# c976237222/HunyuanVideo_efficiency

Hardware: AMD Instinct MI355X
Metric: denoise-steps/sec (720x1280x129f, HunyuanVideo DiT 20+40 blocks, bf16) (higher is better)
Workload: dtype bf16

## Files before the change

hunyuanvideo_efficiency_amd/_lib.py:

```python
from __future__ import annotations

import ctypes as C
import os
import re

_HERE = os.path.dirname(os.path.abspath(__file__))
LIB_PATH = os.path.join(_HERE, "lib", "libhv_kernels.so")
TORCH_OPS_PATH = os.path.join(_HERE, "lib", "libhv_torch_ops.so")
ABI_VERSION = 5

_p, _i, _l, _f = C.c_void_p, C.c_int, C.c_int64, C.c_float

SIGNATURES = {
    "hv_abi_version": [],
    "hv_ln_modulate_bf16": [_p, _p, _p, _p, _l, _i, _l, _l, _f, _i, _p],
    "hv_qknorm_rope_bf16": [_p, _p, _p, _p, _p, _l, _l, _i, _i, _l, _l, _f, _p],
    "hv_qknorm_rope_scatter_bf16": [_p, _p, _p, _p, _p, _l, _l, _i, _i, _l, _l, _f, _p, _l, _i, _l, _p],
    "hv_gemm_bf16": [_p, _l, _p, _l, _p, _i, _i, _i, _p, _l, _i, _i, _p, _l, _i, _p, _p, _l, _p],
    "hv_linear_smallm_bf16": [_p, _p, _p, _p, _p, _i, _i, _i, _l, _l, _i, _p],
    "hv_timestep_embedding_bf16": [_p, _p, _i, _i, _f, _p],
    "hv_attn_fwd_bf16": [_p, _p, _p, _p, _l, _l, _l, _l, _i, _i, _i, _i, _f, _p, _l, _p],
    "hv_attn_workspace_bytes": [_i, _i, _i],
    "hv_attn_w4_loop_signature": [],
    "hv_attn_partial_bf16": [_p, _p, _p, _l, _l, _l, _i, _i, _i, _i, _f, _p, _p, _i, _i, _i, _p],
    "hv_attn_merge_bf16": [_p, _p, _p, _l, _i, _i, _i, _p],
    "hv_attn_suggest_splits": [_i, _i, _i],
    "hv_patchify_f32_bf16": [_p, _p, _i, _i, _i, _i, _p],
    "hv_unpatchify_bf16": [_p, _p, _i, _i, _i, _i, _l, _p],
    "hv_euler_step_f32": [_p, _p, _f, _l, _p],
    "hv_euler_step_f32_f32": [_p, _p, _f, _l, _p],
    "hv_masked_mean_bf16": [_p, _p, _p, _i, _i, _p],
    "hv_broadcast_row_bf16": [_p, _p, _l, _i, _l, _p],
    "hv_copy3d_bf16": [_p, _p, _i, _l, _i, _l, _l, _l, _l, _p],
    "hv_fp8_dequant_bf16": [_p, _p, _p, _l, _p],
    "hv_ln_modulate_fp8": [_p, _p, _p, _p, _p, _l, _i, _l, _l, _f, _p],
    "hv_quant_rows_fp8": [_p, _l, _p, _l, _p, _l, _i, _p],
    "hv_gemm_fp8": [_p, _l, _p, _p, _l, _p, _p, _i, _i, _i, _p, _l, _i, _i, _p, _l, _i, _p, _p, _l, _p],
    "hv_gemm_f16": [_p, _l, _p, _l, _p, _i, _i, _i, _p, _l, _i, _p, _l, _p],
    "hv_conv3d_causal_f16": [_p, _l, _p, _p, _p, _l, _i, _i, _i, _i, _i, _i, _i, _p, _l, _p, _l, _p],
    "hv_gn_partial_rows": [_l],
    "hv_subpixel_gn_partial_rows": [_i, _i, _i, _i],
    "hv_groupnorm_finalize_f16": [_p, _l, _l, _l, _i, _i, _f, _p, _p, _p, _p],
    "hv_groupnorm_affine_f16": [_p, _l, _l, _i, _i, _f, _p, _p, _p, _l, _p, _p],
    "hv_groupnorm_apply_f16": [_p, _l, _p, _l, _l, _i, _p, _i, _p],
    "hv_softmax_rows_f32_f16": [_p, _l, _p, _l, _i, _i, _i, _f, _i, _p],
# ... 91 lines not shown
```

hunyuanvideo_efficiency_amd/csrc/hv_attention.hip:

```cpp
#include "hv_attention.hpp"

using namespace hv_attn;

namespace {

constexpr int QTILE = 256;

__global__ __launch_bounds__(256) void attn_combine_kernel(const float* __restrict__ part_o, const float* __restrict__ part_ml,
                                                            bf16_t* __restrict__ o, int64_t so, int n_q, int n_heads, int n_splits) {
    const int64_t idx = (int64_t)blockIdx.x * blockDim.x + threadIdx.x;
    const int64_t total = (int64_t)n_q * n_heads * 32;
    if (idx >= total) return;
    const int d4 = (int)(idx & 31);
    const int64_t rh = idx >> 5;
    const int head = (int)(rh % n_heads);
    const int64_t row = rh / n_heads;
    float m = -INFINITY;
    for (int s = 0; s < n_splits; ++s) m = fmaxf(m, part_ml[(((int64_t)s * n_q + row) * n_heads + head) * 2]);
    float4 acc = make_float4(0.f, 0.f, 0.f, 0.f);
    float l = 0.f;
    for (int s = 0; s < n_splits; ++s) {
        const int64_t ri = ((int64_t)s * n_q + row) * n_heads + head;
        const float w = __builtin_amdgcn_exp2f(part_ml[ri * 2] - m);
        const float4 v = *reinterpret_cast<const float4*>(part_o + ri * D + d4 * 4);
        acc.x += v.x * w; acc.y += v.y * w; acc.z += v.z * w; acc.w += v.w * w;
        l += part_ml[ri * 2 + 1] * w;
    }
    const float inv = 1.0f / l;
    u32x2 w2;
    w2[0] = pack_bf2(acc.x * inv, acc.y * inv);
    w2[1] = pack_bf2(acc.z * inv, acc.w * inv);
    *reinterpret_cast<u32x2*>(o + row * so + head * D + d4 * 4) = w2;
}

int attn_launch(const AttnArgs& a, dim3 grid, hipStream_t stream) { return launch_w4(a, grid, stream); }

constexpr int KMAX_ROWS = 2048;
__global__ __launch_bounds__(256) void attn_kmax_kernel(const bf16_t* __restrict__ k, int64_t sk, int n_kv, unsigned* __restrict__ out) {
    __shared__ float wmax[4];
    const int head = blockIdx.y, t = threadIdx.x, ch = t & 15;
    const int r0 = blockIdx.x * KMAX_ROWS, r1 = min(r0 + KMAX_ROWS, n_kv);
    float best = 0.f;
    for (int row = r0 + (t >> 4); row < r1; row += 16) {
        const u32x4 w = *reinterpret_cast<const u32x4*>(k + (int64_t)row * sk + head * D + ch * 8);
        float s = 0.f;
#pragma unroll
        for (int j = 0; j < 4; ++j) {
            const float lo = bf2f_lo(w[j]), hi = bf2f_hi(w[j]);
            s += lo * lo + hi * hi;
        }
#pragma unroll
        for (int o = 8; o > 0; o >>= 1) s += __shfl_xor(s, o, 64);
        best = fmaxf(best, s);
    }
    best = fmaxf(best, __shfl_xor(best, 16, 64));
    best = fmaxf(best, __shfl_xor(best, 32, 64));
    if ((t & 63) == 0) wmax[t >> 6] = best;
    __syncthreads();
    if (t == 0) atomicMax(out + head, __float_as_uint(fmaxf(fmaxf(wmax[0], wmax[1]), fmaxf(wmax[2], wmax[3]))));
}

int attn_prepare_kmax(AttnArgs& a, void* workspace, int64_t workspace_bytes, hipStream_t stream) {
    a.kmax2 = nullptr;
    if (!workspace || workspace_bytes < KMAX_BYTES || a.n_heads > KMAX_HEADS || a.n_kv < 64 * KVT) return HV_OK;
    if (hipMemsetAsync(workspace, 0, KMAX_BYTES, stream) != hipSuccess) return HV_ERR_LAUNCH;
    attn_kmax_kernel<<<dim3((unsigned)((a.n_kv + KMAX_ROWS - 1) / KMAX_ROWS), (unsigned)a.n_heads), dim3(256), 0, stream>>>(a.k, a.sk, a.n_kv, (unsigned*)workspace);
    a.kmax2 = (const unsigned*)workspace;
    return HV_OK;
}

}

extern "C" int64_t hv_attn_workspace_bytes(int n_q, int n_kv, int n_heads) {
    (void)n_kv;
    return (int64_t)KMAX_BYTES + (int64_t)2 * n_q * n_heads * (128 + 2) * (int64_t)sizeof(float);
}

extern "C" int hv_attn_fwd_bf16(const void* q, const void* k, const void* v, void* o, int64_t stride_q, int64_t stride_k,
                                int64_t stride_v, int64_t stride_o, int n_q, int n_kv, int n_heads, int head_dim,
                                float scale, void* workspace, int64_t workspace_bytes, hipStream_t stream) {
    if (!q || !k || !v || !o || head_dim != D || n_heads <= 0 || n_q < 0 || n_kv < 0 || (stride_q & 7) || (stride_k & 7) ||
        (stride_v & 7) || (stride_o & 3))
        return HV_ERR_ARG;
    if (n_q == 0) return HV_OK;
    if (n_kv == 0) return HV_ERR_ARG;
    AttnArgs a;
    a.q = (const bf16_t*)q; a.k = (const bf16_t*)k; a.v = (const bf16_t*)v; a.o = (bf16_t*)o;
    a.sq = stride_q; a.sk = stride_k; a.sv = stride_v; a.so = stride_o;
    a.n_q = n_q; a.n_kv = n_kv; a.n_heads = n_heads;
    a.n_qtiles = (n_q + QTILE - 1) / QTILE;
    a.scale_log2e = scale * 1.4426950408889634f;
    a.n_splits = 1; a.split_keys = n_kv; a.part_o = nullptr; a.part_ml = nullptr; a.partial = 0;
    if (attn_prepare_kmax(a, workspace, workspace_bytes, stream) != HV_OK) return HV_ERR_LAUNCH;
    {
        const int64_t nwg = (int64_t)a.n_qtiles * n_heads;
        const int ntile = (n_kv + KVT - 1) / KVT;
        const double r1 = (double)((nwg + 255) / 256), r2 = 0.5 * (double)((2 * nwg + 255) / 256);
        if (workspace && ntile >= 64 && r2 < 0.97 * r1 && workspace_bytes >= hv_attn_workspace_bytes(n_q, n_kv, n_heads)) {
            a.n_splits = 2;
            a.split_keys = ((ntile + 1) / 2) * KVT;
            a.part_o = (float*)((char*)workspace + KMAX_BYTES);
            a.part_ml = a.part_o + (int64_t)2 * n_q * n_heads * D;
        }
    }
    if (attn_launch(a, dim3((unsigned)(a.n_qtiles * n_heads), (unsigned)a.n_splits), stream) != HV_OK) return HV_ERR_LAUNCH;
    if (a.n_splits > 1) {
        const int64_t total = (int64_t)n_q * n_heads * 32;
        attn_combine_kernel<<<dim3((unsigned)((total + 255) / 256)), dim3(256), 0, stream>>>(a.part_o, a.part_ml, a.o, a.so, n_q, n_heads,
                                                                                           a.n_splits);
    }
    return hv_check_launch();
}

extern "C" int hv_attn_partial_bf16(const void* q, const void* k, const void* v, int64_t stride_q, int64_t stride_k, int64_t stride_v,
                                    int n_q, int n_kv, int n_heads, int head_dim, float scale, void* part_o, void* part_ml,
                                    int n_slots, int slot, int splits, hipStream_t stream) {
    if (!q || !k || !v || !part_o || !part_ml || head_dim != D || n_heads <= 0 || n_q < 0 || n_kv <= 0 || (stride_q & 7) ||
        (stride_k & 7) || (stride_v & 7) || (splits != 1 && splits != 2) || slot < 0 || slot + splits > n_slots)
        return HV_ERR_ARG;
    if (n_q == 0) return HV_OK;
    const int ntile = (n_kv + KVT - 1) / KVT;
    if (splits == 2 && ntile < 2) return HV_ERR_ARG;
    AttnArgs a;
    a.q = (const bf16_t*)q; a.k = (const bf16_t*)k; a.v = (const bf16_t*)v; a.o = nullptr;
    a.sq = stride_q; a.sk = stride_k; a.sv = stride_v; a.so = 0;
    a.n_q = n_q; a.n_kv = n_kv; a.n_heads = n_heads;
    a.n_qtiles = (n_q + QTILE - 1) / QTILE;
    a.scale_log2e = scale * 1.4426950408889634f;
    a.n_splits = splits;
    a.split_keys = splits == 2 ? ((ntile + 1) / 2) * KVT : n_kv;
    a.part_o = (float*)part_o + (int64_t)slot * n_q * n_heads * D;
    a.part_ml = (float*)part_ml + (int64_t)slot * n_q * n_heads * 2;
    a.partial = 1;
    a.kmax2 = nullptr;
    if (attn_launch(a, dim3((unsigned)(a.n_qtiles * n_heads), (unsigned)splits), stream) != HV_OK) return HV_ERR_LAUNCH;
    return hv_check_launch();
}

extern "C" int hv_attn_merge_bf16(const void* part_o, const void* part_ml, void* o, int64_t stride_o, int n_q, int n_heads, int n_slots,
                                  hipStream_t stream) {
    if (!part_o || !part_ml || !o || n_heads <= 0 || n_q < 0 || n_slots <= 0 || (stride_o & 3)) return HV_ERR_ARG;
    if (n_q == 0) return HV_OK;
    const int64_t total = (int64_t)n_q * n_heads * 32;
    attn_combine_kernel<<<dim3((unsigned)((total + 255) / 256)), dim3(256), 0, stream>>>((const float*)part_o, (const float*)part_ml,
                                                                                       (bf16_t*)o, stride_o, n_q, n_heads, n_slots);
    return hv_check_launch();
}

extern "C" int hv_attn_suggest_splits(int n_q, int n_kv, int n_heads) {
    const int64_t nwg = (int64_t)((n_q + QTILE - 1) / QTILE) * n_heads;
    const int ntile = (n_kv + KVT - 1) / KVT;
    const double r1 = (double)((nwg + 255) / 256), r2 = 0.5 * (double)((2 * nwg + 255) / 256);
    return (ntile >= 64 && r2 < 0.97 * r1) ? 2 : 1;
}
```

hunyuanvideo_efficiency_amd/csrc/hv_attention.hpp:

```cpp
#pragma once
#include "hv_common.hpp"
#include "../../include/hv_kernels.h"
#include <type_traits>

namespace hv_attn {

constexpr int D = 128;
constexpr int KVT = 64;
constexpr int KV_TILE_BYTES = KVT * D * 2;

struct AttnArgs {
    const bf16_t* q; const bf16_t* k; const bf16_t* v; bf16_t* o;
    int64_t sq, sk, sv, so;
    int n_q, n_kv, n_heads, n_qtiles;
    float scale_log2e;
    int n_splits, split_keys;
    float* part_o;
    float* part_ml;
    int partial;
    const unsigned* kmax2;
};
constexpr int KMAX_BYTES = 256;
constexpr int KMAX_HEADS = 62;

typedef __attribute__((ext_vector_type(4))) short s16x4;
typedef __attribute__((address_space(3))) s16x4* lds_s16x4_ptr;
typedef __attribute__((address_space(3))) void* lds_void_ptr;

__device__ __forceinline__ float half_swap_max(float v) {
    auto r = __builtin_amdgcn_permlane32_swap(__float_as_uint(v), __float_as_uint(v), false, false);
    return fmaxf(__uint_as_float(r[0]), __uint_as_float(r[1]));
}
__device__ __forceinline__ float half_swap_sum(float v) {
    auto r = __builtin_amdgcn_permlane32_swap(__float_as_uint(v), __float_as_uint(v), false, false);
    return __uint_as_float(r[0]) + __uint_as_float(r[1]);
}

template <int I, int N, typename F>
__device__ __forceinline__ void static_for(F&& f) {
    if constexpr (I < N) {
        f(std::integral_constant<int, I>{});
        static_for<I + 1, N>(f);
    }
}

int launch_w4(const AttnArgs& a, dim3 grid, hipStream_t stream);

}
```

hunyuanvideo_efficiency_amd/csrc/hv_attention_w4.hip:

```cpp
#include "hv_attention.hpp"
#include "hv_agpr_clobbers.inc"

using namespace hv_attn;

namespace {

constexpr int W4_WAVES = 4, W4_QTILE = 256, W4_NBUF = 4;
constexpr int W4_KOFF = 0, W4_VOFF = W4_NBUF * KV_TILE_BYTES;
constexpr int W4_LDS = 2 * W4_NBUF * KV_TILE_BYTES;
constexpr int A_O = 0, A_Q = 128, A_KF = 192, A_VF = 224;
constexpr int RING = 8;
constexpr int PF = 4;
constexpr int WGRP = 2;
__host__ __device__ constexpr int frag_insts(int f) { return (f >= 16 && f < 32) ? 2 : 1; }
__host__ __device__ constexpr int wait_for(int f) { int n = 0; for (int i = WGRP; i < PF; ++i) n += frag_insts(f + i); return n; }

template <int KF, int QF, int WAIT>
__device__ __forceinline__ void mfma_s_first(f32x16& s, const f32x16& c) {
    if constexpr (WAIT >= 0)
        asm volatile("s_waitcnt lgkmcnt(%c6)\n\tv_mfma_f32_32x32x16_bf16 %0, a[%c2:%c3], a[%c4:%c5], %1"
                     : "=&v"(s) : "v"(c), "i"(KF), "i"(KF + 3), "i"(QF), "i"(QF + 3), "i"(WAIT) : HV_CLOBBER_ALL_AGPRS);
    else
        asm volatile("v_mfma_f32_32x32x16_bf16 %0, a[%c2:%c3], a[%c4:%c5], %1"
                     : "=&v"(s) : "v"(c), "i"(KF), "i"(KF + 3), "i"(QF), "i"(QF + 3) : HV_CLOBBER_ALL_AGPRS);
// ... 34 lines not shown
__device__ __forceinline__ void add_pinned(float& acc, float p) { asm volatile("v_add_f32 %0, %0, %1" : "+v"(acc) : "v"(p)); }
__device__ __forceinline__ void exp2_pinned(float& d, float x) { asm volatile("v_exp_f32 %0, %1" : "=v"(d) : "v"(x)); }
__device__ __forceinline__ void pack_pinned(uint32_t& w, float lo, float hi) { asm volatile("v_cvt_pk_bf16_f32 %0, %1, %2" : "=v"(w) : "v"(lo), "v"(hi)); }
__device__ __forceinline__ void max3_pinned(float& acc, float x, float y) { asm volatile("v_max3_f32 %0, %0, %1, %2" : "+v"(acc) : "v"(x), "v"(y)); }
template <int N>
__device__ __forceinline__ void acc_write(uint32_t v) { asm volatile("v_accvgpr_write_b32 a%c1, %0" : : "v"(v), "i"(N)); }
template <int N>
__device__ __forceinline__ float acc_read() {
    float v;
    asm volatile("v_accvgpr_read_b32 %0, a%c1" : "=v"(v) : "i"(N));
    return v;
}

#include "hv_attention_w4_loop.inc"

__host__ __device__ constexpr int exps_before(int g) { return g <= 32 ? g + (g + 3) / 4 : (g <= 56 ? 40 + (g - 32) : 64); }
__host__ __device__ constexpr int exps_in(int g) { return exps_before(g + 1) - exps_before(g); }

__global__ __launch_bounds__(256, 1) void attn_fwd_kernel_w4(AttnArgs a) {
#if defined(__HIP_DEVICE_COMPILE__)
    extern __shared__ __attribute__((aligned(16))) char smem[];
    const int tid = threadIdx.x, lane = tid & 63, wave = tid >> 6;
    const int lr = lane & 31, lh = lane >> 5;
    const int head = blockIdx.x / a.n_qtiles;
    const int qt = blockIdx.x % a.n_qtiles;
    if (a.n_splits > 1) {
        const int kv0 = blockIdx.y * a.split_keys;
        a.k += (int64_t)kv0 * a.sk;
        a.v += (int64_t)kv0 * a.sv;
        a.n_kv = min(a.n_kv - kv0, a.split_keys);
    }
    const int q0 = qt * W4_QTILE + wave * 64;
    const uint32_t lds0 = (uint32_t)(uintptr_t)smem;

    asm volatile("; hv_attention_w4: a[0:255] owned by inline asm" : : : HV_CLOBBER_ALL_AGPRS);
    static_for<0, 128>([&](auto I) { asm volatile("v_accvgpr_write_b32 a%c0, 0" : : "i"(A_O + decltype(I)::value)); });
    float qn2[2] = {0.f, 0.f};
#pragma unroll
    for (int qb = 0; qb < 2; ++qb) {
        const int qrow = min(q0 + qb * 32 + lr, a.n_q - 1);
        const bf16_t* qp = a.q + (int64_t)qrow * a.sq + head * D + lh * 8;
        u32x4 raw[8];
#pragma unroll
        for (int ks = 0; ks < 8; ++ks) raw[ks] = *reinterpret_cast<const u32x4*>(qp + ks * 16);
        static_for<0, 32>([&](auto I) {
            constexpr int i = decltype(I)::value;
            const uint32_t w = raw[i >> 2][i & 3];
            const uint32_t sc = pack_bf2(bf2f_lo(w) * a.scale_log2e, bf2f_hi(w) * a.scale_log2e);
            qn2[qb] += bf2f_lo(sc) * bf2f_lo(sc) + bf2f_hi(sc) * bf2f_hi(sc);
            if (qb == 0) acc_write<A_Q + i>(sc);
            else acc_write<A_Q + 32 + i>(sc);
        });
    }

// ... 340 lines not shown
                }
        asm volatile("s_nop 1" : "+v"(pw[0][0]), "+v"(pw[0][1]), "+v"(pw[0][2]), "+v"(pw[0][3]), "+v"(pw[1][0]), "+v"(pw[1][1]), "+v"(pw[1][2]),
                     "+v"(pw[1][3]));
        static_for<0, 16>([&](auto F) {
            constexpr int f = decltype(F)::value, kk = f >> 2, db = f & 3, VF = A_VF + 4 * (f % RING);
            lds_v<VF, kk * 16 * 256>(vv[db]);
            static_for<0, 2>([&](auto QB) {
                constexpr int qb = decltype(QB)::value;
                mfma_pv<A_O + 16 * (qb * 4 + db), VF, (qb == 0 ? 0 : -1)>(pw[qb][kk]);
            });
        });
        l_run[0] += ls[0];
        l_run[1] += ls[1];
    }
    asm volatile("s_nop 7\n\ts_nop 7\n\ts_nop 7" ::: "memory");

#pragma unroll
    for (int qb = 0; qb < 2; ++qb) {
        float o[64];
        if (qb == 0) static_for<0, 64>([&](auto I) { o[decltype(I)::value] = acc_read<A_O + decltype(I)::value>(); });
        else static_for<0, 64>([&](auto I) { o[decltype(I)::value] = acc_read<A_O + 64 + decltype(I)::value>(); });
        const float l_tot = half_swap_sum(l_run[qb]);
        const int qrow = q0 + qb * 32 + lr;
        if (a.n_splits > 1 || a.partial) {
            if (qrow < a.n_q) {
                const int64_t rowi = ((int64_t)blockIdx.y * a.n_q + qrow) * a.n_heads + head;
                float* po = a.part_o + rowi * D + 4 * lh;
#pragma unroll
                for (int db = 0; db < 4; ++db)
#pragma unroll
                    for (int g = 0; g < 4; ++g)
                        *reinterpret_cast<float4*>(po + db * 32 + g * 8) =
                            make_float4(o[db * 16 + 4 * g], o[db * 16 + 4 * g + 1], o[db * 16 + 4 * g + 2], o[db * 16 + 4 * g + 3]);
                if (lh == 0) {
                    a.part_ml[rowi * 2] = m_run[qb];
                    a.part_ml[rowi * 2 + 1] = l_tot;
                }
            }
        } else if (qrow < a.n_q) {
            const float inv = 1.0f / l_tot;
            bf16_t* op = a.o + (int64_t)qrow * a.so + head * D + 4 * lh;
#pragma unroll
            for (int db = 0; db < 4; ++db)
#pragma unroll
                for (int g = 0; g < 4; ++g) {
                    u32x2 w;
                    w[0] = pack_bf2(o[db * 16 + 4 * g] * inv, o[db * 16 + 4 * g + 1] * inv);
                    w[1] = pack_bf2(o[db * 16 + 4 * g + 2] * inv, o[db * 16 + 4 * g + 3] * inv);
                    *reinterpret_cast<u32x2*>(op + db * 32 + g * 8) = w;
                }
        }
    }
#endif
}

HvPerDeviceOnce g_w4_lds_once;

}

extern "C" int hv_attn_w4_loop_signature(void) { return (int)HV_W4_LOOP_SIGNATURE; }

int hv_attn::launch_w4(const AttnArgs& a, dim3 grid, hipStream_t stream) {
    if (hv_set_max_lds(g_w4_lds_once, (const void*)attn_fwd_kernel_w4, W4_LDS) != HV_OK) return HV_ERR_LAUNCH;
    attn_fwd_kernel_w4<<<grid, dim3(256), W4_LDS, stream>>>(a);
    return HV_OK;
}
```

hunyuanvideo_efficiency_amd/csrc/hv_torch_ops.cpp:

```cpp
#include <torch/library.h>
#include <ATen/core/Tensor.h>
#include <c10/hip/HIPStream.h>
#include <c10/hip/HIPGuard.h>
#include <optional>
#include <vector>
#include "../../include/hv_kernels.h"

namespace {
using OptT = std::optional<at::Tensor>;

struct Dev {
    c10::DeviceIndex idx = -1;
    const char* op;
    explicit Dev(const char* o) : op(o) {}
    void* p(const OptT& t, const char* name) {
        if (!t.has_value() || !t->defined()) return nullptr;
        TORCH_CHECK(t->is_cuda(), "hv::", op, ": ", name, " must be a GPU tensor (this library has no CPU path), got ", t->device());
        if (idx < 0) idx = t->device().index();
        TORCH_CHECK(t->device().index() == idx, "hv::", op, ": ", name, " is on a different GPU than the other tensors");
        return t->data_ptr();
    }
};

inline void check_rc(int rc, const char* op) {
// ... 78 lines not shown
    TORCH_CHECK(dev.idx >= 0, "hv::timestep_embedding_bf16: needs at least one GPU tensor");
    c10::hip::HIPGuard guard(dev.idx);
    hipStream_t stream = c10::hip::getCurrentHIPStream(dev.idx).stream();
    check_rc(hv_timestep_embedding_bf16(a0, a1, (int)n_t, (int)dim, (float)max_period, stream), "timestep_embedding_bf16");
}

void op_attn_fwd_bf16(const OptT& q, const OptT& k, const OptT& v, const OptT& o, int64_t stride_q, int64_t stride_k, int64_t stride_v, int64_t stride_o, int64_t n_q, int64_t n_kv, int64_t n_heads, int64_t head_dim, double scale, const OptT& workspace, int64_t workspace_bytes) {
    Dev dev("attn_fwd_bf16");
    auto a0 = (const void*)dev.p(q, "q");
    auto a1 = (const void*)dev.p(k, "k");
    auto a2 = (const void*)dev.p(v, "v");
    auto a3 = (void*)dev.p(o, "o");
    auto a13 = (void*)dev.p(workspace, "workspace");
    TORCH_CHECK(dev.idx >= 0, "hv::attn_fwd_bf16: needs at least one GPU tensor");
    c10::hip::HIPGuard guard(dev.idx);
    hipStream_t stream = c10::hip::getCurrentHIPStream(dev.idx).stream();
    check_rc(hv_attn_fwd_bf16(a0, a1, a2, a3, (int64_t)stride_q, (int64_t)stride_k, (int64_t)stride_v, (int64_t)stride_o, (int)n_q, (int)n_kv, (int)n_heads, (int)head_dim, (float)scale, a13, (int64_t)workspace_bytes, stream), "attn_fwd_bf16");
}

int64_t op_attn_workspace_bytes(int64_t n_q, int64_t n_kv, int64_t n_heads) {
    return (int64_t)hv_attn_workspace_bytes((int)n_q, (int)n_kv, (int)n_heads);
}

int64_t op_attn_w4_loop_signature() {
    return (int64_t)hv_attn_w4_loop_signature();
}

void op_attn_partial_bf16(const OptT& q, const OptT& k, const OptT& v, int64_t stride_q, int64_t stride_k, int64_t stride_v, int64_t n_q, int64_t n_kv, int64_t n_heads, int64_t head_dim, double scale, const OptT& part_o, const OptT& part_ml, int64_t n_slots, int64_t slot, int64_t splits) {
    Dev dev("attn_partial_bf16");
    auto a0 = (const void*)dev.p(q, "q");
    auto a1 = (const void*)dev.p(k, "k");
    auto a2 = (const void*)dev.p(v, "v");
    auto a11 = (void*)dev.p(part_o, "part_o");
    auto a12 = (void*)dev.p(part_ml, "part_ml");
    TORCH_CHECK(dev.idx >= 0, "hv::attn_partial_bf16: needs at least one GPU tensor");
    c10::hip::HIPGuard guard(dev.idx);
    hipStream_t stream = c10::hip::getCurrentHIPStream(dev.idx).stream();
    check_rc(hv_attn_partial_bf16(a0, a1, a2, (int64_t)stride_q, (int64_t)stride_k, (int64_t)stride_v, (int)n_q, (int)n_kv, (int)n_heads, (int)head_dim, (float)scale, a11, a12, (int)n_slots, (int)slot, (int)splits, stream), "attn_partial_bf16");
}

void op_attn_merge_bf16(const OptT& part_o, const OptT& part_ml, const OptT& o, int64_t stride_o, int64_t n_q, int64_t n_heads, int64_t n_slots) {
    Dev dev("attn_merge_bf16");
    auto a0 = (const void*)dev.p(part_o, "part_o");
    auto a1 = (const void*)dev.p(part_ml, "part_ml");
    auto a2 = (void*)dev.p(o, "o");
    TORCH_CHECK(dev.idx >= 0, "hv::attn_merge_bf16: needs at least one GPU tensor");
// ... 314 lines not shown

void op_vae_postprocess_f16_f32(const OptT& x, const OptT& out, int64_t n) {
    Dev dev("vae_postprocess_f16_f32");
    auto a0 = (const void*)dev.p(x, "x");
    auto a1 = (float*)dev.p(out, "out");
    TORCH_CHECK(dev.idx >= 0, "hv::vae_postprocess_f16_f32: needs at least one GPU tensor");
    c10::hip::HIPGuard guard(dev.idx);
    hipStream_t stream = c10::hip::getCurrentHIPStream(dev.idx).stream();
    check_rc(hv_vae_postprocess_f16_f32(a0, a1, (int64_t)n, stream), "vae_postprocess_f16_f32");
}

}

TORCH_LIBRARY(hv, m) {
    m.def("abi_version() -> int");
    m.def("ln_modulate_bf16(Tensor? x, Tensor? shift_or_bias, Tensor? scale_or_weight, Tensor(a!)? out, int M, int D, int ldx, int ldo, float eps, int mode) -> ()");
    m.def("qknorm_rope_bf16(Tensor(a!)? qkv, Tensor? q_weight, Tensor? k_weight, Tensor? cos_tab, Tensor? sin_tab, int n_rows, int n_rope, int n_heads, int head_dim, int ld, int k_offset, float eps) -> ()");
    m.def("qknorm_rope_scatter_bf16(Tensor? qkv, Tensor? q_weight, Tensor? k_weight, Tensor? cos_tab, Tensor? sin_tab, int n_rows, int n_rope, int n_heads, int head_dim, int ld, int k_offset, float eps, Tensor(a!)? dst, int dst_ld, int heads_per_block, int dst_block_stride) -> ()");
    m.def("gemm_bf16(Tensor? A, int lda, Tensor? W, int ldw, Tensor? bias, int M, int N, int K, Tensor(a!)? out0, int ld0, int act0, int n_split, Tensor(b!)? out1, int ld1, int act1, Tensor? gate, Tensor? res, int ld_res) -> ()");
    m.def("linear_smallm_bf16(Tensor? x, Tensor? W, Tensor? bias, Tensor? addend, Tensor(a!)? out, int M, int N, int K, int ldx, int ldo, int act) -> ()");
    m.def("timestep_embedding_bf16(Tensor? t, Tensor(a!)? out, int n_t, int dim, float max_period) -> ()");
    m.def("attn_fwd_bf16(Tensor? q, Tensor? k, Tensor? v, Tensor(a!)? o, int stride_q, int stride_k, int stride_v, int stride_o, int n_q, int n_kv, int n_heads, int head_dim, float scale, Tensor(b!)? workspace, int workspace_bytes) -> ()");
    m.def("attn_workspace_bytes(int n_q, int n_kv, int n_heads) -> int");
    m.def("attn_w4_loop_signature() -> int");
    m.def("attn_partial_bf16(Tensor? q, Tensor? k, Tensor? v, int stride_q, int stride_k, int stride_v, int n_q, int n_kv, int n_heads, int head_dim, float scale, Tensor(a!)? part_o, Tensor(b!)? part_ml, int n_slots, int slot, int splits) -> ()");
    m.def("attn_merge_bf16(Tensor? part_o, Tensor? part_ml, Tensor(a!)? o, int stride_o, int n_q, int n_heads, int n_slots) -> ()");
    m.def("attn_suggest_splits(int n_q, int n_kv, int n_heads) -> int");
    m.def("patchify_f32_bf16(Tensor? x, Tensor(a!)? A, int C, int T, int H, int W) -> ()");
    m.def("unpatchify_bf16(Tensor? y, Tensor(a!)? out, int C, int T, int H, int W, int ldy) -> ()");
    m.def("euler_step_f32(Tensor(a!)? sample, Tensor? model_out_bf16, float dt, int n) -> ()");
    m.def("euler_step_f32_f32(Tensor(a!)? sample, Tensor? model_out_f32, float dt, int n) -> ()");
    m.def("masked_mean_bf16(Tensor? x, Tensor? mask, Tensor(a!)? out, int L, int D) -> ()");
    m.def("broadcast_row_bf16(Tensor? src, Tensor(a!)? dst, int n_rows, int D, int ld) -> ()");
    m.def("copy3d_bf16(Tensor? src, Tensor(a!)? dst, int n_batch, int rows, int cols, int src_batch_stride, int src_ld, int dst_batch_stride, int dst_ld) -> ()");
    m.def("fp8_dequant_bf16(Tensor? w_e4m3fn, Tensor? scale_bf16, Tensor(a!)? out_bf16, int n) -> ()");
    m.def("ln_modulate_fp8(Tensor? x, Tensor? shift, Tensor? scale, Tensor(a!)? out_q, Tensor(b!)? out_row_scale, int M, int D, int ldx, int ldq, float eps) -> ()");
    m.def("quant_rows_fp8(Tensor? x, int ldx, Tensor(a!)? out_q, int ldq, Tensor(b!)? out_row_scale, int M, int K) -> ()");
    m.def("gemm_fp8(Tensor? A_q, int lda, Tensor? a_row_scale, Tensor? W_q, int ldw, Tensor? w_scale_bf16, Tensor? bias, int M, int N, int K, Tensor(a!)? out0, int ld0, int act0, int n_split, Tensor(b!)? out1, int ld1, int act1, Tensor? gate, Tensor? res, int ld_res) -> ()");
    m.def("gemm_f16(Tensor? A, int lda, Tensor? W, int ldw, Tensor? bias, int M, int N, int K, Tensor(a!)? out, int ldo, int out_is_f32, Tensor? res, int ld_res) -> ()");
    m.def("conv3d_causal_f16(Tensor? x, int ldx, Tensor? w_taps, Tensor? bias, Tensor(a!)? out, int ldo, int T, int H, int W, int Cin, int Cout, int up_t, int up_hw, Tensor? res, int ld_res, Tensor(b!)? gn_partial, int gn_partial_floats) -> ()");
    m.def("gn_partial_rows(int M) -> int");
    m.def("subpixel_gn_partial_rows(int sT, int sH, int sW, int up_t) -> int");
    m.def("conv3d_upsampled_subpixel_f16(Tensor? x, int ldx, Tensor? w_sub, Tensor? tap_table, int ntap, Tensor? bias, Tensor(a!)? out, int ldo, int sT, int sH, int sW, int Cin, int Cout, int up_t, Tensor(b!)? gn_partial, int gn_partial_floats) -> ()");
    m.def("conv3d_cout4_f16(Tensor? x, int ldx, Tensor? affine, int silu, Tensor? w_frag, Tensor? bias, Tensor(a!)? out, int ldo, int T, int H, int W, int Cin, int Cout, Tensor(b!)? planes, int planes_floats) -> ()");
    m.def("conv3d_cout4_planes_floats(int M) -> int");
    m.def("conv3d_causal_strided_f16(Tensor? x, int ldx, Tensor? w_taps, Tensor? bias, Tensor(a!)? out, int ldo, int sT, int sH, int sW, int Cin, int Cout, int stride_t, int stride_h, int stride_w) -> ()");
// ... 30 lines not shown
    m.impl("ln_modulate_fp8", &op_ln_modulate_fp8);
    m.impl("quant_rows_fp8", &op_quant_rows_fp8);
    m.impl("gemm_fp8", &op_gemm_fp8);
    m.impl("gemm_f16", &op_gemm_f16);
    m.impl("conv3d_causal_f16", &op_conv3d_causal_f16);
    m.impl("conv3d_upsampled_subpixel_f16", &op_conv3d_upsampled_subpixel_f16);
    m.impl("conv3d_cout4_f16", &op_conv3d_cout4_f16);
    m.impl("conv3d_causal_strided_f16", &op_conv3d_causal_strided_f16);
    m.impl("temporal_resample_f16", &op_temporal_resample_f16);
    m.impl("groupnorm_affine_f16", &op_groupnorm_affine_f16);
    m.impl("groupnorm_finalize_f16", &op_groupnorm_finalize_f16);
    m.impl("groupnorm_apply_f16", &op_groupnorm_apply_f16);
    m.impl("softmax_rows_f32_f16", &op_softmax_rows_f32_f16);
    m.impl("transpose_16b", &op_transpose_16b);
    m.impl("vae_latent_tile_f16", &op_vae_latent_tile_f16);
    m.impl("vae_blend_f16", &op_vae_blend_f16);
    m.impl("copy4d_16b", &op_copy4d_16b);
    m.impl("vae_postprocess_f16_f32", &op_vae_postprocess_f16_f32);
}

TORCH_LIBRARY_IMPL(hv, CompositeExplicitAutograd, m) {
    m.impl("abi_version", &op_abi_version);
    m.impl("attn_workspace_bytes", &op_attn_workspace_bytes);
    m.impl("attn_w4_loop_signature", &op_attn_w4_loop_signature);
    m.impl("attn_suggest_splits", &op_attn_suggest_splits);
    m.impl("gn_partial_rows", &op_gn_partial_rows);
    m.impl("subpixel_gn_partial_rows", &op_subpixel_gn_partial_rows);
    m.impl("conv3d_cout4_planes_floats", &op_conv3d_cout4_planes_floats);
}
```

hunyuanvideo_efficiency_amd/ops.py:

```python
from __future__ import annotations

from typing import Optional

import torch

from . import _lib

BF16 = torch.bfloat16
ACT_NONE, ACT_GELU_TANH, ACT_SILU = 0, 1, 2
PROFILE_ATTN = None


def _chk(t: torch.Tensor, dtype, name: str, last_contig: bool = True):
    if not t.is_cuda:
        raise _lib.HVKernelError(f"{name}: expected a GPU tensor (this package has no CPU path), got {t.device}")
    if t.dtype != dtype:
        raise TypeError(f"{name}: expected {dtype}, got {t.dtype}")
    if last_contig and t.dim() > 0 and t.stride(-1) != 1:
        raise ValueError(f"{name}: innermost dimension must be contiguous")


def _rows(t: torch.Tensor, name: str):
    if t.dim() == 1:
        return 1, t.shape[0], t.shape[0]
# ... 82 lines not shown
    assert k == kw and ldw == k and m <= 4
    if out is None:
        out = torch.empty(*x.shape[:-1], n, dtype=BF16, device=x.device)
    _, _, ldo = _rows(out, "out")
    if bias is not None:
        _chk(bias, BF16, "bias")
    if addend is not None:
        _chk(addend, BF16, "addend")
        assert addend.shape == out.shape and addend.stride() == out.stride()
    _lib.call("linear_smallm_bf16", x, w, bias, addend, out, m, n, k, ldx, ldo,
                                                 (1 if silu_in else 0) | (2 if silu_out else 0))
    return out


_attn_ws = {}


ATTN_MIN_WORKSPACE = 256


def _attn_workspace(n_q, n_kv, n_heads, device):
    if n_kv < 64 * 64:
        return None
    n_wg = ((n_q + 255) // 256) * n_heads
    need = ATTN_MIN_WORKSPACE if n_wg >= 16 * 256 else int(_lib.host("attn_workspace_bytes", n_q, n_kv, n_heads))
    key = str(device)
    ws = _attn_ws.get(key)
    if ws is None or ws.numel() < need:
        ws = torch.empty(need, dtype=torch.uint8, device=device)
        _attn_ws[key] = ws
    return ws


def attn_fwd(q, k, v, out, n_heads: int, scale: Optional[float] = None, kv_split_workspace: bool = True):
    for t, nm in ((q, "q"), (k, "k"), (v, "v"), (out, "out")):
        _chk(t, BF16, nm)
        assert t.dim() == 2
    n_q, n_kv = q.shape[0], k.shape[0]
    assert v.shape[0] == n_kv and out.shape[0] == n_q
    if scale is None:
        scale = 128 ** -0.5
    prof = PROFILE_ATTN
    if prof is not None:
        e0, e1 = torch.cuda.Event(enable_timing=True), torch.cuda.Event(enable_timing=True)
        e0.record()
    ws = _attn_workspace(n_q, n_kv, n_heads, q.device) if kv_split_workspace else None
    _lib.call("attn_fwd_bf16", q, k, v, out, q.stride(0), k.stride(0), v.stride(0),
                                            out.stride(0), n_q, n_kv, n_heads, 128, scale, ws,
# ... 184 lines not shown
```

include/hv_kernels.h:

```cpp
#ifndef HV_KERNELS_H
#define HV_KERNELS_H

#include <stdint.h>

#ifdef __cplusplus
extern "C" {
#endif

#ifndef __HIP__
typedef struct ihipStream_t* hipStream_t;
#endif

int hv_abi_version(void);

int hv_ln_modulate_bf16(const void* x, const void* shift_or_bias, const void* scale_or_weight, void* out,
                        int64_t M, int D, int64_t ldx, int64_t ldo, float eps, int mode, hipStream_t stream);

int hv_qknorm_rope_bf16(void* qkv, const void* q_weight, const void* k_weight, const float* cos_tab,
                        const float* sin_tab, int64_t n_rows, int64_t n_rope, int n_heads, int head_dim,
                        int64_t ld, int64_t k_offset, float eps, hipStream_t stream);

int hv_qknorm_rope_scatter_bf16(const void* qkv, const void* q_weight, const void* k_weight, const float* cos_tab,
                                const float* sin_tab, int64_t n_rows, int64_t n_rope, int n_heads, int head_dim, int64_t ld,
                                int64_t k_offset, float eps, void* dst, int64_t dst_ld, int heads_per_block,
                                int64_t dst_block_stride, hipStream_t stream);

int hv_gemm_bf16(const void* A, int64_t lda, const void* W, int64_t ldw, const void* bias, int M, int N, int K,
                 void* out0, int64_t ld0, int act0, int n_split, void* out1, int64_t ld1, int act1,
                 const void* gate, const void* res, int64_t ld_res, hipStream_t stream);

int hv_linear_smallm_bf16(const void* x, const void* W, const void* bias, const void* addend, void* out, int M,
                          int N, int K, int64_t ldx, int64_t ldo, int act, hipStream_t stream);

int hv_timestep_embedding_bf16(const float* t, void* out, int n_t, int dim, float max_period, hipStream_t stream);

#define HV_ATTN_MIN_WORKSPACE_BYTES 256
int hv_attn_fwd_bf16(const void* q, const void* k, const void* v, void* o, int64_t stride_q, int64_t stride_k,
                     int64_t stride_v, int64_t stride_o, int n_q, int n_kv, int n_heads, int head_dim,
                     float scale, void* workspace, int64_t workspace_bytes, hipStream_t stream);

int64_t hv_attn_workspace_bytes(int n_q, int n_kv, int n_heads);
int hv_attn_w4_loop_signature(void);

int hv_attn_partial_bf16(const void* q, const void* k, const void* v, int64_t stride_q, int64_t stride_k, int64_t stride_v,
                         int n_q, int n_kv, int n_heads, int head_dim, float scale, void* part_o, void* part_ml,
                         int n_slots, int slot, int splits, hipStream_t stream);

int hv_attn_merge_bf16(const void* part_o, const void* part_ml, void* o, int64_t stride_o, int n_q, int n_heads, int n_slots,
                       hipStream_t stream);

int hv_attn_suggest_splits(int n_q, int n_kv, int n_heads);

int hv_patchify_f32_bf16(const float* x, void* A, int C, int T, int H, int W, hipStream_t stream);

int hv_unpatchify_bf16(const void* y, void* out, int C, int T, int H, int W, int64_t ldy, hipStream_t stream);

int hv_euler_step_f32(float* sample, const void* model_out_bf16, float dt, int64_t n, hipStream_t stream);

int hv_euler_step_f32_f32(float* sample, const float* model_out_f32, float dt, int64_t n, hipStream_t stream);

int hv_masked_mean_bf16(const void* x, const int* mask, void* out, int L, int D, hipStream_t stream);

int hv_broadcast_row_bf16(const void* src, void* dst, int64_t n_rows, int D, int64_t ld, hipStream_t stream);

// ... 74 lines not shown
```

Before: 0.1168.

## Split only tail-wave attention work items across KV to balance CUs

Measured after the change: 0.1173 (median of 6 runs). No clear change (+0.5%).

```diff
diff --git a/hunyuanvideo_efficiency_amd/_lib.py b/hunyuanvideo_efficiency_amd/_lib.py
--- a/hunyuanvideo_efficiency_amd/_lib.py
+++ b/hunyuanvideo_efficiency_amd/_lib.py
@@ -21,6 +21,7 @@
     "hv_timestep_embedding_bf16": [_p, _p, _i, _i, _f, _p],
     "hv_attn_fwd_bf16": [_p, _p, _p, _p, _l, _l, _l, _l, _i, _i, _i, _i, _f, _p, _l, _p],
     "hv_attn_workspace_bytes": [_i, _i, _i],
+    "hv_attn_tail_splits": [_i, _i, _i, _i, _l],
     "hv_attn_w4_loop_signature": [],
     "hv_attn_partial_bf16": [_p, _p, _p, _l, _l, _l, _i, _i, _i, _i, _f, _p, _p, _i, _i, _i, _p],
     "hv_attn_merge_bf16": [_p, _p, _p, _l, _i, _i, _i, _p],
diff --git a/hunyuanvideo_efficiency_amd/csrc/hv_attention.hip b/hunyuanvideo_efficiency_amd/csrc/hv_attention.hip
--- a/hunyuanvideo_efficiency_amd/csrc/hv_attention.hip
+++ b/hunyuanvideo_efficiency_amd/csrc/hv_attention.hip
@@ -5,6 +5,26 @@
 namespace {
 
 constexpr int QTILE = 256;
+
+__device__ __forceinline__ u32x2 combine_row(const float* __restrict__ part_o, const float* __restrict__ part_ml, int64_t ri0, int64_t ri_step,
+                                             int n_pieces, int d4) {
+    float m = -INFINITY;
+    for (int s = 0; s < n_pieces; ++s) m = fmaxf(m, part_ml[(ri0 + s * ri_step) * 2]);
+    float4 acc = make_float4(0.f, 0.f, 0.f, 0.f);
+    float l = 0.f;
+    for (int s = 0; s < n_pieces; ++s) {
+        const int64_t ri = ri0 + s * ri_step;
+        const float w = __builtin_amdgcn_exp2f(part_ml[ri * 2] - m);
+        const float4 v = *reinterpret_cast<const float4*>(part_o + ri * D + d4 * 4);
+        acc.x += v.x * w; acc.y += v.y * w; acc.z += v.z * w; acc.w += v.w * w;
+        l += part_ml[ri * 2 + 1] * w;
+    }
+    const float inv = 1.0f / l;
+    u32x2 w2;
+    w2[0] = pack_bf2(acc.x * inv, acc.y * inv);
+    w2[1] = pack_bf2(acc.z * inv, acc.w * inv);
+    return w2;
+}
 
 __global__ __launch_bounds__(256) void attn_combine_kernel(const float* __restrict__ part_o, const float* __restrict__ part_ml,
                                                             bf16_t* __restrict__ o, int64_t so, int n_q, int n_heads, int n_splits) {
@@ -15,25 +35,24 @@
     const int64_t rh = idx >> 5;
     const int head = (int)(rh % n_heads);
     const int64_t row = rh / n_heads;
-    float m = -INFINITY;
-    for (int s = 0; s < n_splits; ++s) m = fmaxf(m, part_ml[(((int64_t)s * n_q + row) * n_heads + head) * 2]);
-    float4 acc = make_float4(0.f, 0.f, 0.f, 0.f);
-    float l = 0.f;
-    for (int s = 0; s < n_splits; ++s) {
-        const int64_t ri = ((int64_t)s * n_q + row) * n_heads + head;
-        const float w = __builtin_amdgcn_exp2f(part_ml[ri * 2] - m);
-        const float4 v = *reinterpret_cast<const float4*>(part_o + ri * D + d4 * 4);
-        acc.x += v.x * w; acc.y += v.y * w; acc.z += v.z * w; acc.w += v.w * w;
-        l += part_ml[ri * 2 + 1] * w;
-    }
-    const float inv = 1.0f / l;
-    u32x2 w2;
-    w2[0] = pack_bf2(acc.x * inv, acc.y * inv);
-    w2[1] = pack_bf2(acc.z * inv, acc.w * inv);
-    *reinterpret_cast<u32x2*>(o + row * so + head * D + d4 * 4) = w2;
-}
-
-int attn_launch(const AttnArgs& a, dim3 grid, hipStream_t stream) { return launch_w4(a, grid, stream); }
+    *reinterpret_cast<u32x2*>(o + row * so + head * D + d4 * 4) = combine_row(part_o, part_ml, rh, (int64_t)n_q * n_heads, n_splits, d4);
+}
+
+__global__ __launch_bounds__(256) void attn_tail_combine_kernel(const float* __restrict__ part_o, const float* __restrict__ part_ml,
+                                                                 bf16_t* __restrict__ o, int64_t so, int n_q, int n_qtiles, int n_whole,
+                                                                 int n_tail, int n_splits) {
+    const int64_t idx = (int64_t)blockIdx.x * blockDim.x + threadIdx.x;
+    if (idx >= (int64_t)n_tail * QTILE * 32) return;
+    const int d4 = (int)(idx & 31);
+    const int j = (int)(idx >> 5) / QTILE, lrow = (int)(idx >> 5) % QTILE;
+    const int item = n_whole + j, head = item / n_qtiles;
+    const int64_t row = (int64_t)(item % n_qtiles) * QTILE + lrow;
+    if (row >= n_q) return;
+    *reinterpret_cast<u32x2*>(o + row * so + head * D + d4 * 4) =
+        combine_row(part_o, part_ml, (int64_t)j * n_splits * QTILE + lrow, QTILE, n_splits, d4);
+}
+
+int attn_launch(const AttnArgs& a, int64_t n_wg, hipStream_t stream) { return launch_w4(a, n_wg, stream); }
 
 constexpr int KMAX_ROWS = 2048;
 __global__ __launch_bounds__(256) void attn_kmax_kernel(const bf16_t* __restrict__ k, int64_t sk, int n_kv, unsigned* __restrict__ out) {
@@ -69,11 +88,57 @@
     return HV_OK;
 }
 
+constexpr int TAIL_MAX_SPLITS = 8;
+constexpr int TAIL_MIN_TILES = 32;
+constexpr int FALLBACK_CUS = 256;
+
+struct TailPlan {
+    int splits = 1;
+    int64_t n_tail = 0;
+    int64_t bytes = 0;
+};
+
+TailPlan attn_tail_plan(int n_q, int n_kv, int n_heads, int n_cus) {
+    TailPlan p;
+    if (n_q <= 0 || n_kv <= 0 || n_heads <= 0 || n_cus <= 0) return p;
+    const int64_t items = (int64_t)((n_q + QTILE - 1) / QTILE) * n_heads;
+    const int64_t r = items % n_cus;
+    const int ntile = (n_kv + KVT - 1) / KVT;
+    if (r == 0) return p;
+    int64_t best_rounds = 1;
+    for (int s = 2; s <= TAIL_MAX_SPLITS && ntile >= s * TAIL_MIN_TILES; ++s) {
+        const int64_t rounds = (r * s + n_cus - 1) / n_cus;
+        if (rounds * p.splits < best_rounds * s) { best_rounds = rounds; p.splits = s; }
+    }
+    if (p.splits > 1) {
+        p.n_tail = r;
+        p.bytes = r * p.splits * QTILE * (D + 2) * (int64_t)sizeof(float);
+    }
+    return p;
+}
+
+int attn_device_cus() {
+    static int cus[64] = {};
+    int dev = 0;
+    if (hipGetDevice(&dev) != hipSuccess || dev < 0 || dev >= 64) return 0;
+    if (cus[dev] <= 0) {
+        int n = 0;
+        if (hipDeviceGetAttribute(&n, hipDeviceAttributeMultiprocessorCount, dev) != hipSuccess) return 0;
+        cus[dev] = n;
+    }
+    return cus[dev];
+}
+
 }
 
 extern "C" int64_t hv_attn_workspace_bytes(int n_q, int n_kv, int n_heads) {
-    (void)n_kv;
-    return (int64_t)KMAX_BYTES + (int64_t)2 * n_q * n_heads * (128 + 2) * (int64_t)sizeof(float);
+    const int cus = attn_device_cus();
+    return (int64_t)KMAX_BYTES + attn_tail_plan(n_q, n_kv, n_heads, cus > 0 ? cus : FALLBACK_CUS).bytes;
+}
+
+extern "C" int hv_attn_tail_splits(int n_q, int n_kv, int n_heads, int n_cus, int64_t workspace_bytes) {
+    const TailPlan p = attn_tail_plan(n_q, n_kv, n_heads, n_cus);
+    return workspace_bytes >= (int64_t)KMAX_BYTES + p.bytes ? p.splits : 1;
 }
 
 extern "C" int hv_attn_fwd_bf16(const void* q, const void* k, const void* v, void* o, int64_t stride_q, int64_t stride_k,
@@ -90,25 +155,26 @@
     a.n_q = n_q; a.n_kv = n_kv; a.n_heads = n_heads;
     a.n_qtiles = (n_q + QTILE - 1) / QTILE;
     a.scale_log2e = scale * 1.4426950408889634f;
-    a.n_splits = 1; a.split_keys = n_kv; a.part_o = nullptr; a.part_ml = nullptr; a.partial = 0;
+    const int64_t items = (int64_t)a.n_qtiles * n_heads;
+    a.n_whole = (int)items; a.n_splits = 1; a.split_keys = n_kv; a.part_o = nullptr; a.part_ml = nullptr; a.partial = 0;
     if (attn_prepare_kmax(a, workspace, workspace_bytes, stream) != HV_OK) return HV_ERR_LAUNCH;
-    {
-        const int64_t nwg = (int64_t)a.n_qtiles * n_heads;
+    TailPlan tail;
+    if (workspace) {
+        tail = attn_tail_plan(n_q, n_kv, n_heads, attn_device_cus());
+        if (workspace_bytes < (int64_t)KMAX_BYTES + tail.bytes) tail = TailPlan();
+    }
+    if (tail.splits > 1) {
         const int ntile = (n_kv + KVT - 1) / KVT;
-        const double r1 = (double)((nwg + 255) / 256), r2 = 0.5 * (double)((2 * nwg + 255) / 256);
-        if (workspace && ntile >= 64 && r2 < 0.97 * r1 && workspace_bytes >= hv_attn_workspace_bytes(n_q, n_kv, n_heads)) {
-            a.n_splits = 2;
-            a.split_keys = ((ntile + 1) / 2) * KVT;
-            a.part_o = (float*)((char*)workspace + KMAX_BYTES);
-            a.part_ml = a.part_o + (int64_t)2 * n_q * n_heads * D;
-        }
-    }
-    if (attn_launch(a, dim3((unsigned)(a.n_qtiles * n_heads), (unsigned)a.n_splits), stream) != HV_OK) return HV_ERR_LAUNCH;
-    if (a.n_splits > 1) {
-        const int64_t total = (int64_t)n_q * n_heads * 32;
-        attn_combine_kernel<<<dim3((unsigned)((total + 255) / 256)), dim3(256), 0, stream>>>(a.part_o, a.part_ml, a.o, a.so, n_q, n_heads,
-                                                                                           a.n_splits);
-    }
+        a.n_whole = (int)(items - tail.n_tail);
+        a.n_splits = tail.splits;
+        a.split_keys = ((ntile + tail.splits - 1) / tail.splits) * KVT;
+        a.part_o = (float*)((char*)workspace + KMAX_BYTES);
+        a.part_ml = a.part_o + tail.n_tail * tail.splits * QTILE * D;
+    }
+    if (attn_launch(a, a.n_whole + tail.n_tail * tail.splits, stream) != HV_OK) return HV_ERR_LAUNCH;
+    if (tail.splits > 1)
+        attn_tail_combine_kernel<<<dim3((unsigned)(tail.n_tail * QTILE * 32 / 256)), dim3(256), 0, stream>>>(
+            a.part_o, a.part_ml, a.o, a.so, n_q, a.n_qtiles, a.n_whole, (int)tail.n_tail, tail.splits);
     return hv_check_launch();
 }
 
@@ -127,13 +193,14 @@
     a.n_q = n_q; a.n_kv = n_kv; a.n_heads = n_heads;
     a.n_qtiles = (n_q + QTILE - 1) / QTILE;
     a.scale_log2e = scale * 1.4426950408889634f;
+    a.n_whole = 0;
     a.n_splits = splits;
     a.split_keys = splits == 2 ? ((ntile + 1) / 2) * KVT : n_kv;
     a.part_o = (float*)part_o + (int64_t)slot * n_q * n_heads * D;
     a.part_ml = (float*)part_ml + (int64_t)slot * n_q * n_heads * 2;
     a.partial = 1;
     a.kmax2 = nullptr;
-    if (attn_launch(a, dim3((unsigned)(a.n_qtiles * n_heads), (unsigned)splits), stream) != HV_OK) return HV_ERR_LAUNCH;
+    if (attn_launch(a, (int64_t)a.n_qtiles * n_heads * splits, stream) != HV_OK) return HV_ERR_LAUNCH;
     return hv_check_launch();
 }
 
diff --git a/hunyuanvideo_efficiency_amd/csrc/hv_attention.hpp b/hunyuanvideo_efficiency_amd/csrc/hv_attention.hpp
--- a/hunyuanvideo_efficiency_amd/csrc/hv_attention.hpp
+++ b/hunyuanvideo_efficiency_amd/csrc/hv_attention.hpp
@@ -14,7 +14,7 @@
     int64_t sq, sk, sv, so;
     int n_q, n_kv, n_heads, n_qtiles;
     float scale_log2e;
-    int n_splits, split_keys;
+    int n_whole, n_splits, split_keys;
     float* part_o;
     float* part_ml;
     int partial;
@@ -44,6 +44,6 @@
     }
 }
 
-int launch_w4(const AttnArgs& a, dim3 grid, hipStream_t stream);
+int launch_w4(const AttnArgs& a, int64_t n_wg, hipStream_t stream);
 
 }
diff --git a/hunyuanvideo_efficiency_amd/csrc/hv_attention_w4.hip b/hunyuanvideo_efficiency_amd/csrc/hv_attention_w4.hip
--- a/hunyuanvideo_efficiency_amd/csrc/hv_attention_w4.hip
+++ b/hunyuanvideo_efficiency_amd/csrc/hv_attention_w4.hip
@@ -80,14 +80,19 @@
     extern __shared__ __attribute__((aligned(16))) char smem[];
     const int tid = threadIdx.x, lane = tid & 63, wave = tid >> 6;
     const int lr = lane & 31, lh = lane >> 5;
-    const int head = blockIdx.x / a.n_qtiles;
-    const int qt = blockIdx.x % a.n_qtiles;
-    if (a.n_splits > 1) {
-        const int kv0 = blockIdx.y * a.split_keys;
+    const int wg = blockIdx.x;
+    const bool piece = wg >= a.n_whole;
+    int item = wg, split = 0;
+    if (piece) {
+        item = a.n_whole + (wg - a.n_whole) / a.n_splits;
+        split = (wg - a.n_whole) % a.n_splits;
+        const int kv0 = split * a.split_keys;
         a.k += (int64_t)kv0 * a.sk;
         a.v += (int64_t)kv0 * a.sv;
         a.n_kv = min(a.n_kv - kv0, a.split_keys);
     }
+    const int head = item / a.n_qtiles;
+    const int qt = item % a.n_qtiles;
     const int q0 = qt * W4_QTILE + wave * 64;
     const uint32_t lds0 = (uint32_t)(uintptr_t)smem;
 
@@ -474,9 +479,10 @@
         else static_for<0, 64>([&](auto I) { o[decltype(I)::value] = acc_read<A_O + 64 + decltype(I)::value>(); });
         const float l_tot = half_swap_sum(l_run[qb]);
         const int qrow = q0 + qb * 32 + lr;
-        if (a.n_splits > 1 || a.partial) {
+        if (piece) {
             if (qrow < a.n_q) {
-                const int64_t rowi = ((int64_t)blockIdx.y * a.n_q + qrow) * a.n_heads + head;
+                const int64_t rowi = a.partial ? ((int64_t)split * a.n_q + qrow) * a.n_heads + head
+                                               : ((int64_t)(item - a.n_whole) * a.n_splits + split) * W4_QTILE + (qrow - qt * W4_QTILE);
                 float* po = a.part_o + rowi * D + 4 * lh;
 #pragma unroll
                 for (int db = 0; db < 4; ++db)
@@ -512,8 +518,9 @@
 
 extern "C" int hv_attn_w4_loop_signature(void) { return (int)HV_W4_LOOP_SIGNATURE; }
 
-int hv_attn::launch_w4(const AttnArgs& a, dim3 grid, hipStream_t stream) {
+int hv_attn::launch_w4(const AttnArgs& a, int64_t n_wg, hipStream_t stream) {
+    if (n_wg <= 0 || n_wg > INT32_MAX) return HV_ERR_ARG;
     if (hv_set_max_lds(g_w4_lds_once, (const void*)attn_fwd_kernel_w4, W4_LDS) != HV_OK) return HV_ERR_LAUNCH;
-    attn_fwd_kernel_w4<<<grid, dim3(256), W4_LDS, stream>>>(a);
+    attn_fwd_kernel_w4<<<dim3((unsigned)n_wg), dim3(256), W4_LDS, stream>>>(a);
     return HV_OK;
 }
diff --git a/hunyuanvideo_efficiency_amd/csrc/hv_torch_ops.cpp b/hunyuanvideo_efficiency_amd/csrc/hv_torch_ops.cpp
--- a/hunyuanvideo_efficiency_amd/csrc/hv_torch_ops.cpp
+++ b/hunyuanvideo_efficiency_amd/csrc/hv_torch_ops.cpp
@@ -124,6 +124,10 @@
     return (int64_t)hv_attn_workspace_bytes((int)n_q, (int)n_kv, (int)n_heads);
 }
 
+int64_t op_attn_tail_splits(int64_t n_q, int64_t n_kv, int64_t n_heads, int64_t n_cus, int64_t workspace_bytes) {
+    return (int64_t)hv_attn_tail_splits((int)n_q, (int)n_kv, (int)n_heads, (int)n_cus, (int64_t)workspace_bytes);
+}
+
 int64_t op_attn_w4_loop_signature() {
     return (int64_t)hv_attn_w4_loop_signature();
 }
@@ -484,6 +488,7 @@
     m.def("timestep_embedding_bf16(Tensor? t, Tensor(a!)? out, int n_t, int dim, float max_period) -> ()");
     m.def("attn_fwd_bf16(Tensor? q, Tensor? k, Tensor? v, Tensor(a!)? o, int stride_q, int stride_k, int stride_v, int stride_o, int n_q, int n_kv, int n_heads, int head_dim, float scale, Tensor(b!)? workspace, int workspace_bytes) -> ()");
     m.def("attn_workspace_bytes(int n_q, int n_kv, int n_heads) -> int");
+    m.def("attn_tail_splits(int n_q, int n_kv, int n_heads, int n_cus, int workspace_bytes) -> int");
     m.def("attn_w4_loop_signature() -> int");
     m.def("attn_partial_bf16(Tensor? q, Tensor? k, Tensor? v, int stride_q, int stride_k, int stride_v, int n_q, int n_kv, int n_heads, int head_dim, float scale, Tensor(a!)? part_o, Tensor(b!)? part_ml, int n_slots, int slot, int splits) -> ()");
     m.def("attn_merge_bf16(Tensor? part_o, Tensor? part_ml, Tensor(a!)? o, int stride_o, int n_q, int n_heads, int n_slots) -> ()");
@@ -560,6 +565,7 @@
 TORCH_LIBRARY_IMPL(hv, CompositeExplicitAutograd, m) {
     m.impl("abi_version", &op_abi_version);
     m.impl("attn_workspace_bytes", &op_attn_workspace_bytes);
+    m.impl("attn_tail_splits", &op_attn_tail_splits);
     m.impl("attn_w4_loop_signature", &op_attn_w4_loop_signature);
     m.impl("attn_suggest_splits", &op_attn_suggest_splits);
     m.impl("gn_partial_rows", &op_gn_partial_rows);
diff --git a/hunyuanvideo_efficiency_amd/ops.py b/hunyuanvideo_efficiency_amd/ops.py
--- a/hunyuanvideo_efficiency_amd/ops.py
+++ b/hunyuanvideo_efficiency_amd/ops.py
@@ -128,8 +128,7 @@
 def _attn_workspace(n_q, n_kv, n_heads, device):
     if n_kv < 64 * 64:
         return None
-    n_wg = ((n_q + 255) // 256) * n_heads
-    need = ATTN_MIN_WORKSPACE if n_wg >= 16 * 256 else int(_lib.host("attn_workspace_bytes", n_q, n_kv, n_heads))
+    need = max(ATTN_MIN_WORKSPACE, int(_lib.host("attn_workspace_bytes", n_q, n_kv, n_heads)))
     key = str(device)
     ws = _attn_ws.get(key)
     if ws is None or ws.numel() < need:
diff --git a/include/hv_kernels.h b/include/hv_kernels.h
--- a/include/hv_kernels.h
+++ b/include/hv_kernels.h
@@ -40,6 +40,7 @@
                      float scale, void* workspace, int64_t workspace_bytes, hipStream_t stream);
 
 int64_t hv_attn_workspace_bytes(int n_q, int n_kv, int n_heads);
+int hv_attn_tail_splits(int n_q, int n_kv, int n_heads, int n_cus, int64_t workspace_bytes);
 int hv_attn_w4_loop_signature(void);
 
 int hv_attn_partial_bf16(const void* q, const void* k, const void* v, int64_t stride_q, int64_t stride_k, int64_t stride_v,
```
